# Healthcare-Robotics/assistive-gym

Hardware: NVIDIA H100
Metric: env-steps/sec FeedingJaco-v1 @batch4096 (higher is better)
Workload: dtype f32

## Files before the change

assistive_gym_b200/csrc/ag_bathing.cuh:

```cuda
#pragma once
#include "ag_task.cuh"
#include "../../include/agphys.h"

struct BathDev {
  AgBathingParams P;
  int *male, *iteration, *task_success, *total_targets;
  float* action;
  float* targets;
  int* alive;
  int* target_link;
  float* target_local;
  float* dist_part;
  int n_slots;
};

AG_HDN inline void bathing_pre_body(int e, const SimDev& S, const KP& p) {
  const BathDev& B = *(const BathDev*)p.p1;
  const float* act = (const float*)p.p0 + (size_t)e * (7 + p.i0);
  B.iteration[e] += 1;
  arm_action_targets(S, e, act, B.action, B.P.arm_links, B.P.arm_lower, B.P.arm_upper, B.P.action_multiplier, B.P.frame_skip);
}

AG_HDN inline void bathing_dist_body(int tid, const SimDev& S, const KP& p) {
  const int N = S.N;
  const BathDev& B = *(const BathDev*)p.p1;
  int e = tid % N, slot = tid / N;
  bool male = B.male[e] != 0;
  int c0 = male ? B.P.human_col0_m : B.P.human_col0_f, nc = male ? B.P.human_ncol_m : B.P.human_ncol_f;
  float best = 5.0f;
  if (slot < nc) {
    int ch = c0 + slot;
    int lt = AG_LDG(S.body_link0 + B.P.tool_body), nlt = AG_LDG(S.body_nlinks + B.P.tool_body);
    for (int l = lt; l < lt + nlt; l++) {
      int t0 = AG_LDG(S.link_col0 + l), tn = AG_LDG(S.link_ncol + l);
      for (int ct = t0; ct < t0 + tn; ct++) {
        NpOut out[4];
        int ca = ct < ch ? ct : ch, cb = ct < ch ? ch : ct;
        if (narrow_pair(S, e, ca, cb, 5.0f, false, out)) best = fminf(best, out[0].d);
      }
    }
  }
  B.dist_part[(size_t)slot * N + e] = best;
}

AG_HDN inline void bathing_track_body(int tid, const SimDev& S, const KP& p) {
  const int N = S.N;
  const BathDev& B = *(const BathDev*)p.p1;
  const int e = tid % N, t = tid / N;
  const int link = B.target_link[(size_t)t * N + e];
  if (link < 0) return;
  st3(B.targets, t, N, e, ld3(S.lpos, link, N, e) + qrot(ld4(S.lquat, link, N, e), ld3(B.target_local, t, N, e)));
}

// ... 49 lines not shown
```

assistive_gym_b200/csrc/ag_device.cuh:

```cuda
#pragma once
#include <string.h>
#include "ag_math.cuh"
#include "ag_types.h"

AG_HD float ld1(const float* p, int item, int N, int e) { return p[(size_t)item * N + e]; }
AG_HD void st1(float* p, int item, int N, int e, float v) { p[(size_t)item * N + e] = v; }
AG_HD f3 ld3(const float* p, int item, int N, int e) {
  size_t b = (size_t)item * 3 * N + e;
  return f3(p[b], p[b + N], p[b + 2 * (size_t)N]);
}
AG_HD void st3(float* p, int item, int N, int e, f3 v) {
  size_t b = (size_t)item * 3 * N + e;
  p[b] = v.x; p[b + N] = v.y; p[b + 2 * (size_t)N] = v.z;
}
AG_HD q4 ld4(const float* p, int item, int N, int e) {
  size_t b = (size_t)item * 4 * N + e;
  return q4(p[b], p[b + N], p[b + 2 * (size_t)N], p[b + 3 * (size_t)N]);
}
AG_HD void st4(float* p, int item, int N, int e, q4 v) {
  size_t b = (size_t)item * 4 * N + e;
  p[b] = v.x; p[b + N] = v.y; p[b + 2 * (size_t)N] = v.z; p[b + 3 * (size_t)N] = v.w;
}
AG_HD f3 tv3(const float* p, int i) { return f3(AG_LDG(p + 3 * i), AG_LDG(p + 3 * i + 1), AG_LDG(p + 3 * i + 2)); }
AG_HD q4 tv4(const float* p, int i) { return q4(AG_LDG(p + 4 * i), AG_LDG(p + 4 * i + 1), AG_LDG(p + 4 * i + 2), AG_LDG(p + 4 * i + 3)); }
// ... 50 lines not shown
  f3 hw(fabsf(R.m[0]) * h.x + fabsf(R.m[1]) * h.y + fabsf(R.m[2]) * h.z + r,
        fabsf(R.m[3]) * h.x + fabsf(R.m[4]) * h.y + fabsf(R.m[5]) * h.z + r,
        fabsf(R.m[6]) * h.x + fabsf(R.m[7]) * h.y + fabsf(R.m[8]) * h.z + r);
  st3(S.cmin, c, N, e, ctr - hw); st3(S.cmax, c, N, e, ctr + hw);
}
AG_HDN inline void linkaabb_body(int tid, const SimDev& S, const KP& p) {
  const int N = S.N;
  int e = tid % N, i = tid / N;
  int k = AG_LDG((const int*)p.p0 + i);
  int c0 = AG_LDG(S.link_col0 + k), ncl = AG_LDG(S.link_ncol + k);
  f3 mn(1e30f, 1e30f, 1e30f), mx(-1e30f, -1e30f, -1e30f);
  for (int c = c0; c < c0 + ncl; c++) { mn = fmin3(mn, ld3(S.cmin, c, N, e)); mx = fmax3(mx, ld3(S.cmax, c, N, e)); }
  st3(S.lmin, k, N, e, mn); st3(S.lmax, k, N, e, mx);
}

AG_HD bool aabb_ov(f3 amin, f3 amax, f3 bmin, f3 bmax, float m) {
  return !(amin.x > bmax.x + m || bmin.x > amax.x + m || amin.y > bmax.y + m || bmin.y > amax.y + m ||
           amin.z > bmax.z + m || bmin.z > amax.z + m);
}

AG_HD void seg_origin(d3 a, d3 b, double& u, double& v) {
  d3 ab = b - a;
  double t = -dot(a, ab), den = dot(ab, ab);
  if (t <= 0.0 || den <= 0.0) { u = 1.0; v = 0.0; return; }
  if (t >= den) { u = 0.0; v = 1.0; return; }
  v = t / den; u = 1.0 - v;
}
AG_HD void tri_origin(d3 a, d3 b, d3 c, double& u, double& v, double& w) {
  d3 ab = b - a, ac = c - a;
  double d1 = -dot(ab, a), d2 = -dot(ac, a);
// ... 26 lines not shown
  int bi = 0; float best = -3.0e38f;
  const int ng = (n + 3) >> 2;
  const float* p = vq + (size_t)g0 * 12;
  for (int g = 0; g < ng; g++, p += 12) {
    vq4 X = ldq4(p), Y = ldq4(p + 4), Z = ldq4(p + 8);
    float d0 = d.x * X.x + d.y * Y.x + d.z * Z.x, d1 = d.x * X.y + d.y * Y.y + d.z * Z.y;
    float d2 = d.x * X.z + d.y * Y.z + d.z * Z.z, d3v = d.x * X.w + d.y * Y.w + d.z * Z.w;
    if (d0 > best) { best = d0; bi = 4 * g; }
    if (d1 > best) { best = d1; bi = 4 * g + 1; }
    if (d2 > best) { best = d2; bi = 4 * g + 2; }
    if (d3v > best) { best = d3v; bi = 4 * g + 3; }
  }
  return bi < n ? bi : 0;
}

AG_HDN inline bool gjk_cores(const float* verts, const float* vq, int va0, int ga0, int nA, int vb0, int gb0, int nB, const m3& R, f3 t,
                             f3& pa, f3& pb, f3& nrm, float& dist) {
  d3 W[4]; f3 PA[4], PB[4];
  int IA[4], IB[4];
  double lam[4] = {1.0, 0.0, 0.0, 0.0};
  int n = 0;
  d3 v = to_d3(mul(R, tv3(verts, va0)) + t) - to_d3(tv3(verts, vb0));
  if (dot(v, v) < 1e-20) v = d3(1.0, 0.0, 0.0);
  bool overlap = false;
  double lower_bound = 0.0;
  for (int it = 0; it < 32; it++) {
    f3 vf = to_f3(v);
    f3 da = mulT(R, -vf);
    int ia = support4(vq, ga0, nA, da), ib = support4(vq, gb0, nB, vf);
    f3 sa = mul(R, tv3(verts, va0 + ia)) + t;
    f3 sb = tv3(verts, vb0 + ib);
    d3 w = to_d3(sa) - to_d3(sb);
    double vv = dot(v, v);
    double vw = dot(v, w);
    if (n > 0 && vw > 0.0) lower_bound = fmax(lower_bound, vw / sqrt(vv));
    if (n > 0 && vv - vw <= 1e-10 * vv) break;
    bool dup = false;
    for (int i = 0; i < n; i++) if (IA[i] == ia && IB[i] == ib) dup = true;
    if (dup) break;
    W[n] = w; PA[n] = sa; PB[n] = sb; IA[n] = ia; IB[n] = ib; n++;
    if (n == 1) { lam[0] = 1.0; }
    else if (n == 2) {
      double u, s; seg_origin(W[0], W[1], u, s);
      if (s <= 0.0) { n = 1; lam[0] = 1.0; }
      else if (u <= 0.0) { W[0] = W[1]; PA[0] = PA[1]; PB[0] = PB[1]; IA[0] = IA[1]; IB[0] = IB[1]; n = 1; lam[0] = 1.0; }
      else { lam[0] = u; lam[1] = s; }
    } else if (n == 3) {
      double l3[3]; tri_origin(W[0], W[1], W[2], l3[0], l3[1], l3[2]);
      int m = 0;
      for (int i = 0; i < 3; i++) if (l3[i] > 0.0) { W[m] = W[i]; PA[m] = PA[i]; PB[m] = PB[i]; IA[m] = IA[i]; IB[m] = IB[i]; lam[m] = l3[i]; m++; }
      n = m;
    } else {
      double bestd = 1e300; int bf = -1; double bl[3] = {0.0, 0.0, 0.0};
      double bestd_all = 1e300; int bf_all = 0; double bla[3] = {1.0, 0.0, 0.0};
      bool any_out = false;
      for (int f = 0; f < 4; f++) {
        int i0 = (f == 3) ? 1 : 0, i1 = (f == 0) ? 1 : ((f == 1) ? 2 : 3), i2 = (f == 0) ? 2 : ((f == 1) ? 3 : ((f == 2) ? 1 : 2)), i3 = (f == 0) ? 3 : ((f == 1) ? 1 : ((f == 2) ? 2 : 0));
        d3 a = W[i0], b = W[i1], c = W[i2], d = W[i3];
        d3 nn = cross(b - a, c - a);
        double sp = -dot(a, nn), sd = dot(d - a, nn);
        double nl = sqrt(dot(nn, nn));
        double tol_d = 1e-9 * nl * sqrt(dot(d - a, d - a)), tol_p = 1e-9 * nl * sqrt(dot(a, a));
        bool inside = (sp * sd > 0.0) && (fabs(sd) > tol_d) && (fabs(sp) > tol_p);
        double u, s, r; tri_origin(a, b, c, u, s, r);
        d3 pt = a * u + b * s + c * r;
        double dd = dot(pt, pt);
        if (dd < bestd_all) { bestd_all = dd; bf_all = f; bla[0] = u; bla[1] = s; bla[2] = r; }
        if (inside) continue;
        any_out = true;
        if (dd < bestd) { bestd = dd; bf = f; bl[0] = u; bl[1] = s; bl[2] = r; }
      }
      if (!any_out) {
        if (lower_bound <= 1e-7) { overlap = true; break; }
        bf = bf_all; bl[0] = bla[0]; bl[1] = bla[1]; bl[2] = bla[2];
      }
      int f = bf;
      int id[3];
      id[0] = (f == 3) ? 1 : 0; id[1] = (f == 0) ? 1 : ((f == 1) ? 2 : 3); id[2] = (f == 0) ? 2 : ((f == 1) ? 3 : ((f == 2) ? 1 : 2));
      d3 tw[3]; f3 ta[3], tb[3]; int tia[3], tib[3];
      for (int i = 0; i < 3; i++) { tw[i] = W[id[i]]; ta[i] = PA[id[i]]; tb[i] = PB[id[i]]; tia[i] = IA[id[i]]; tib[i] = IB[id[i]]; }
      int m = 0;
      for (int i = 0; i < 3; i++) if (bl[i] > 0.0) { W[m] = tw[i]; PA[m] = ta[i]; PB[m] = tb[i]; IA[m] = tia[i]; IB[m] = tib[i]; lam[m] = bl[i]; m++; }
      n = m;
    }
    d3 nv(0.0, 0.0, 0.0);
    for (int i = 0; i < n; i++) nv = nv + W[i] * lam[i];
    v = nv;
    if (dot(v, v) <= 1e-16) { overlap = true; break; }
  }
  if (overlap) return true;
  d3 qa(0.0, 0.0, 0.0), qb(0.0, 0.0, 0.0);
  for (int i = 0; i < n; i++) { qa = qa + to_d3(PA[i]) * lam[i]; qb = qb + to_d3(PB[i]) * lam[i]; }
  d3 d = qa - qb;
  double dn = sqrt(dot(d, d));
  pa = to_f3(qa); pb = to_f3(qb);
  dist = (float)dn;
  nrm = dn > 0.0 ? to_f3(d * (1.0 / dn)) : f3(0.f, 0.f, 1.f);
  return false;
}

AG_HDN inline void pen_faces(const SimDev& S, int va0, int nA, int pa0, int npA, int vb0, int nB, int pb0, int npB,
                             const m3& R, f3 t, f3& pa, f3& pb, f3& nrm, float& dist) {
  float best = -1e30f; bool found = false;
  for (int k = 0; k < npA; k++) {
    f3 nl; float dl; ld_plane(S.planes, pa0 + k, nl, dl);
    f3 n = mul(R, nl); float d = dl + dot(n, t);
    int jb = 0; float mn = dot(n, tv3(S.verts, vb0));
// ... 1 lines not shown
    float sep = mn - d;
    if (sep > best) { best = sep; found = true; nrm = -n; pb = tv3(S.verts, vb0 + jb); pa = pb - n * sep; }
  }
  for (int k = 0; k < npB; k++) {
    f3 n; float d; ld_plane(S.planes, pb0 + k, n, d);
    f3 nl = mulT(R, n);
    int ja = 0; float mn = dot(nl, tv3(S.verts, va0));
    for (int j = 1; j < nA; j++) { float x = dot(nl, tv3(S.verts, va0 + j)); if (x < mn) { mn = x; ja = j; } }
    float sep = mn + dot(n, t) - d;
    if (sep > best) { best = sep; found = true; nrm = n; pa = mul(R, tv3(S.verts, va0 + ja)) + t; pb = pa - n * sep; }
  }
  if (!found) { nrm = f3(0.f, 0.f, 1.f); pa = mul(R, tv3(S.verts, va0)) + t; pb = tv3(S.verts, vb0); best = 0.f; }
  dist = fminf(best, 0.f);
}

struct CandSet { NpOut c[4]; int n; };
struct CandSel {
  NpOut prim; NpOut pool[12]; int np;
};

AG_HDN inline void face_cands(const SimDev& S, int vv0, int nV, float rV, bool v_is_a, int p0, int np, float rP,
                              const m3& R, f3 t, f3 n_to_v, float d_primary, float tol, float max_dist, CandSel& cs) {
  int kf = -1; float best = 0.98f; f3 nf; float df = 0.f;
  for (int k = 0; k < np; k++) {
    f3 n; float d; ld_plane(S.planes, p0 + k, n, d);
    if (!v_is_a) { f3 nw = mul(R, n); d = d + dot(nw, t); n = nw; }
    float al = dot(n, n_to_v);
    if (al > best) { best = al; kf = k; nf = n; df = d; }
  }
  if (kf < 0) return;
  for (int i = 0; i < nV; i++) {
    f3 v = tv3(S.verts, vv0 + i);
    if (v_is_a) v = mul(R, v) + t;
    float h = dot(nf, v) - df;
    float d = h - rV - rP;
    if (d > d_primary + tol || d > max_dist) continue;
    f3 proj = v - nf * h;
    bool inside = true;
    for (int k = 0; k < np; k++) {
      if (k == kf) continue;
      f3 n; float dd; ld_plane(S.planes, p0 + k, n, dd);
      if (!v_is_a) { f3 nw = mul(R, n); dd = dd + dot(nw, t); n = nw; }
      if (dot(n, proj) - dd > 1e-6f) { inside = false; break; }
    }
    if (!inside) continue;
    if (cs.np >= 12) {
      int wi = 0; for (int q = 1; q < 12; q++) if (cs.pool[q].d > cs.pool[wi].d) wi = q;
      if (d >= cs.pool[wi].d) continue;
      cs.np = 12;
      NpOut& o = cs.pool[wi];
      f3 on_v = v - nf * rV, on_f = proj + nf * rP;
      if (v_is_a) { o.pa = on_v; o.pb = on_f; o.n = nf; } else { o.pa = on_f; o.pb = on_v; o.n = -nf; }
      o.d = d;
      continue;
    }
    NpOut& o = cs.pool[cs.np++];
    f3 on_v = v - nf * rV, on_f = proj + nf * rP;
    if (v_is_a) { o.pa = on_v; o.pb = on_f; o.n = nf; } else { o.pa = on_f; o.pb = on_v; o.n = -nf; }
    o.d = d;
  }
}

AG_HDN inline int select_cands(const CandSel& cs, NpOut* out) {
  if (cs.np == 0) { out[0] = cs.prim; return 1; }
  bool used[12];
  int first = 0;
  for (int i = 0; i < 12; i++) used[i] = i >= cs.np;
  for (int i = 1; i < cs.np; i++) if (cs.pool[i].d < cs.pool[first].d) first = i;
  int nc = 0; out[nc++] = cs.pool[first]; used[first] = true;
  while (nc < 4) {
    int bi = -1; float bd = 1e-8f;
    for (int i = 0; i < cs.np; i++) {
      if (used[i]) continue;
      float md = 1e30f;
      for (int k = 0; k < nc; k++) { f3 d = cs.pool[i].pa - out[k].pa; md = fminf(md, dot(d, d)); }
      if (md > bd) { bd = md; bi = i; }
    }
    if (bi < 0) break;
    used[bi] = true; out[nc++] = cs.pool[bi];
  }
  return nc;
}

AG_HDN inline int narrow_pair(const SimDev& S, int e, int ca, int cb, float max_dist, bool manifold, NpOut* out) {
  const int N = S.N;
  int ta = AG_LDG(S.col_type + ca), tb = AG_LDG(S.col_type + cb);
  float ra = AG_LDG(S.col_radius + ca), rb = AG_LDG(S.col_radius + cb);
  int ka = AG_LDG(S.col_link + ca), kb = AG_LDG(S.col_link + cb);
  int va0 = AG_LDG(S.col_v0 + ca), nA = AG_LDG(S.col_nv + ca), vb0 = AG_LDG(S.col_v0 + cb), nB = AG_LDG(S.col_nv + cb);
  int pa0 = AG_LDG(S.col_p0 + ca), npA = AG_LDG(S.col_np + ca), pb0 = AG_LDG(S.col_p0 + cb), npB = AG_LDG(S.col_np + cb);
  f3 posA = ld3(S.lpos, ka, N, e), posB = ld3(S.lpos, kb, N, e);
  q4 qA = ld4(S.lquat, ka, N, e), qB = ld4(S.lquat, kb, N, e);
  CandSel cs; cs.np = 0;
  int nout;
  if (ta == 3 || tb == 3) {
    if (ta == tb) return 0;
    bool flip = (ta == 3);
    q4 qP = flip ? qA : qB, qV = flip ? qB : qA;
    f3 pP = flip ? posA : posB, pV = flip ? posB : posA;
    m3 R = mul(transpose(qmat(qP)), qmat(qV));
    f3 t = qrot_inv(qP, pV - pP);
    int vv0 = flip ? vb0 : va0, nV = flip ? nB : nA; float rv = flip ? rb : ra;
    f3 pn; float pd; ld_plane(S.planes, flip ? pa0 : pb0, pn, pd);
    int j = 0; float mn = 1e30f;
    for (int i = 0; i < nV; i++) { float x = dot(pn, mul(R, tv3(S.verts, vv0 + i)) + t); if (x < mn) { mn = x; j = i; } }
    float d = mn - pd - rv;
    if (d > max_dist) return 0;
    f3 vj = mul(R, tv3(S.verts, vv0 + j)) + t;
    cs.prim.pa = vj - pn * rv; cs.prim.pb = vj - pn * (mn - pd); cs.prim.n = pn; cs.prim.d = d;
    if (manifold && nV > 1) face_cands(S, vv0, nV, rv, true, flip ? pa0 : pb0, 1, 0.f, R, t, pn, d, max_dist * 0.5f, max_dist, cs);
    nout = select_cands(cs, out);
    m3 RP = qmat(qP);
    for (int i = 0; i < nout; i++) {
      f3 a = mul(RP, out[i].pa) + pP, b = mul(RP, out[i].pb) + pP, n = mul(RP, out[i].n);
      if (!flip) { out[i].pa = a; out[i].pb = b; out[i].n = n; }
      else { out[i].pa = b; out[i].pb = a; out[i].n = -n; }
    }
    return nout;
  }
  m3 RB = qmat(qB);
  m3 R = mul(transpose(RB), qmat(qA));
  f3 t = mulT(RB, posA - posB);
  f3 pa, pb, nrm; float dist = 0.f;
  bool ov = gjk_cores(S.verts, S.vertq, va0, AG_LDG(S.col_g0 + ca), nA, vb0, AG_LDG(S.col_g0 + cb), nB, R, t, pa, pb, nrm, dist);
  if (ov) pen_faces(S, va0, nA, pa0, npA, vb0, nB, pb0, npB, R, t, pa, pb, nrm, dist);
  float d = dist - ra - rb;
  if (d > max_dist) return 0;
  cs.prim.n = nrm; cs.prim.pa = pa - nrm * ra; cs.prim.pb = pb + nrm * rb; cs.prim.d = d;
  if (manifold) {
    if (npB > 0 && nA > 1) face_cands(S, va0, nA, ra, true, pb0, npB, rb, R, t, nrm, d, max_dist * 0.5f, max_dist, cs);
    if (npA > 0 && nB > 1) face_cands(S, vb0, nB, rb, false, pa0, npA, ra, R, t, -nrm, d, max_dist * 0.5f, max_dist, cs);
  }
  nout = select_cands(cs, out);
  for (int i = 0; i < nout; i++) {
    out[i].pa = mul(RB, out[i].pa) + posB; out[i].pb = mul(RB, out[i].pb) + posB; out[i].n = mul(RB, out[i].n);
  }
  return nout;
}

AG_HD int ag_atomic_inc(int* p) {
#if defined(__CUDA_ARCH__)
  return atomicAdd(p, 1);
#else
  int v = *p; *p = v + 1; return v;
#endif
}
AG_HD int ag_atomic_add(int* p, int k) {
#if defined(__CUDA_ARCH__)
  return atomicAdd(p, k);
#else
  int v = *p; *p = v + k; return v;
#endif
// ... 25 lines not shown
    }
  }
}

AG_HDN inline void csort_body(int tid, const SimDev& S, const KP&) {
  const int N = S.N;
  int e = tid % N, cs = tid / N;
  int n = S.cand_count[e]; if (n > S.maxcand) n = S.maxcand;
  if (cs >= n) return;
  unsigned w = S.cand[(size_t)cs * N + e];
  int rank = 0;
  for (int j = 0; j < n; j++) rank += (S.cand[(size_t)j * N + e] < w) ? 1 : 0;
  S.cand_s[(size_t)rank * N + e] = w;
}

AG_HDN inline void narrow_body(int tid, const SimDev& S, const KP&) {
  const int N = S.N;
  int e = tid % N, cs = tid / N;
  int ncand = S.cand_count[e]; if (ncand > S.maxcand) ncand = S.maxcand;
  if (cs >= ncand) return;
  unsigned pk = S.cand_s[(size_t)cs * N + e] & 0xffffffu;
  int ca = (int)(pk / (unsigned)S.nc), cb = (int)(pk % (unsigned)S.nc);
  float thr = S.contact_thr * fminf(AG_LDG(S.col_thresh + ca), AG_LDG(S.col_thresh + cb));
  NpOut out[4];
  int n = narrow_pair(S, e, ca, cb, thr, true, out);
  for (int i = 0; i < n; i++) {
    int slot = ag_atomic_inc(S.c_count + e);
    if (slot >= S.maxraw) continue;
    S.c_key[(size_t)slot * N + e] = pk * 4u + (unsigned)i;
    float* c = S.c_data + (size_t)slot * AG_CFR * N + e;
    c[(size_t)CF_PAX * N] = out[i].pa.x; c[(size_t)CF_PAY * N] = out[i].pa.y; c[(size_t)CF_PAZ * N] = out[i].pa.z;
    c[(size_t)CF_PBX * N] = out[i].pb.x; c[(size_t)CF_PBY * N] = out[i].pb.y; c[(size_t)CF_PBZ * N] = out[i].pb.z;
    c[(size_t)CF_NX * N] = out[i].n.x; c[(size_t)CF_NY * N] = out[i].n.y; c[(size_t)CF_NZ * N] = out[i].n.z;
    c[(size_t)CF_DIST * N] = out[i].d;
  }
}

AG_HD void contact_refs(const SimDev& S, int e, unsigned key, int& refA, int& refB);
AG_HDN inline void sort_body(int tid, const SimDev& S, const KP&) {
  const int N = S.N;
  int e = tid % N, slot = tid / N;
  int cnt = S.c_count[e];
  int n = cnt < S.maxraw ? cnt : S.maxraw;
  if (slot == 0 && ((cnt > S.maxc) || (S.cand_count[e] > S.maxcand))) S.overflow[e] = 1;
  if (slot >= n) return;
  unsigned key = S.c_key[(size_t)slot * N + e];
  int rank = 0;
  for (int j = 0; j < n; j++) rank += (S.c_key[(size_t)j * N + e] < key) ? 1 : 0;
  if (rank >= S.maxc) return;
  S.s_key[(size_t)rank * N + e] = key;
// ... 248 lines not shown
```

assistive_gym_b200/csrc/ag_readback.cuh:

```cuda
#pragma once
#include <string.h>
#include "ag_task.cuh"

AG_HDN inline void gather_body(int tid, const SimDev& S, const KP& p) {
  const int N = S.N;
  int e = tid % N, j = tid / N;
  int comp = p.i0, K = p.i0 * p.i1;
  int item = ((const int*)p.p2)[j / comp], c = j % comp;
  ((float*)p.p1)[(size_t)e * K + j] = ((const float*)p.p0)[((size_t)item * comp + c) * N + e];
}
AG_HDN inline void scatter_body(int tid, const SimDev& S, const KP& p) {
  const int N = S.N;
  int e = tid % N, j = tid / N;
  if (p.p3 && !((const int*)p.p3)[e]) return;
  int comp = p.i0, K = p.i0 * p.i1;
  int item = ((const int*)p.p2)[j / comp], c = j % comp;
  ((float*)p.p1)[((size_t)item * comp + c) * N + e] = ((const float*)p.p0)[(size_t)e * K + j];
}

AG_HDN inline void linkstate_body(int tid, const SimDev& S, const KP& p) {
  const int N = S.N;
  int e = tid % N, j = tid / N, n = p.i1;
  int k = ((const int*)p.p2)[j];
  float* o = (float*)p.p1 + ((size_t)e * n + j) * 20;
// ... 47 lines not shown
  int ba = p.i0, bb = p.i1, max_pts = p.i2; float dist = p.f0;
  int a0 = AG_LDG(S.body_link0 + ba), an = AG_LDG(S.body_nlinks + ba), b0 = AG_LDG(S.body_link0 + bb), bn = AG_LDG(S.body_nlinks + bb);
  int n = 0;
  if (S.body_mode[(size_t)ba * N + e] == 0 || S.body_mode[(size_t)bb * N + e] == 0) { ((int*)p.p2)[e] = 0; return; }
  for (int la = a0; la < a0 + an; la++) {
    int nca = AG_LDG(S.link_ncol + la); if (!nca) continue;
    f3 lamin = ld3(S.lmin, la, N, e), lamax = ld3(S.lmax, la, N, e);
    for (int lb = b0; lb < b0 + bn; lb++) {
      int ncb = AG_LDG(S.link_ncol + lb); if (!ncb) continue;
      if (!aabb_ov(lamin, lamax, ld3(S.lmin, lb, N, e), ld3(S.lmax, lb, N, e), dist)) continue;
      int ca0 = AG_LDG(S.link_col0 + la), cb0 = AG_LDG(S.link_col0 + lb);
      for (int ca = ca0; ca < ca0 + nca; ca++) {
        f3 amin = ld3(S.cmin, ca, N, e), amax = ld3(S.cmax, ca, N, e);
        for (int cb = cb0; cb < cb0 + ncb; cb++) {
          if (!aabb_ov(amin, amax, ld3(S.cmin, cb, N, e), ld3(S.cmax, cb, N, e), dist)) continue;
          NpOut out[4];
          if (!narrow_pair(S, e, ca, cb, dist, false, out)) continue;
          if (n < max_pts) write_contact((float*)p.p1 + ((size_t)e * max_pts + n) * 13, la, lb, out[0].pa, out[0].pb, out[0].n, out[0].d, 0.f);
          n++;
        }
      }
    }
  }
  ((int*)p.p2)[e] = n;
}
```

assistive_gym_b200/csrc/ag_task.cuh:

```cuda
#pragma once
#include "ag_device.cuh"

AG_HD unsigned long long xorshift64s(unsigned long long& s) {
  s ^= s >> 12; s ^= s << 25; s ^= s >> 27;
  return s * 2685821657736338717ull;
}
AG_HD float rng_uniform(unsigned long long& s) { return (float)(xorshift64s(s) >> 40) * (1.0f / 16777216.0f); }

AG_HD void link_com_pose(const SimDev& S, int e, int k, f3& pos, q4& quat) {
  const int N = S.N;
  q4 q = ld4(S.lquat, k, N, e);
  pos = ld3(S.lpos, k, N, e) + qrot(q, tv3(S.link_com, k));
  quat = qmul(q, tv4(S.link_iquat, k));
}
AG_HD f3 link_com(const SimDev& S, int e, int k) {
  const int N = S.N;
  return ld3(S.lpos, k, N, e) + qrot(ld4(S.lquat, k, N, e), tv3(S.link_com, k));
}

struct Frame { f3 p; q4 qi; };
AG_HD Frame body_frame(const SimDev& S, int e, int body) {
  Frame fr; q4 q;
  link_com_pose(S, e, AG_LDG(S.body_link0 + body), fr.p, q);
  fr.qi = qconj(q);
// ... 101 lines not shown
  const int N = S.N;
  float an = 0.f;
  for (int j = 0; j < 7; j++) { float a = action[(size_t)j * N + e]; an += a * a; }
  for (int j = 0; j < i0; j++) { float a = act[(size_t)e * (7 + i0) + 7 + j]; an += a * a; }
  return sqrtf(an);
}
AG_HD float episode_done(int iteration) { return iteration >= 200 ? 1.f : 0.f; }

AG_HD bool tool_within(const SimDev& S, int e, int col, int tool_link, float dist) {
  const int N = S.N;
  f3 pmin = ld3(S.cmin, col, N, e), pmax = ld3(S.cmax, col, N, e);
  if (!aabb_ov(pmin, pmax, ld3(S.lmin, tool_link, N, e), ld3(S.lmax, tool_link, N, e), dist)) return false;
  int c0 = AG_LDG(S.link_col0 + tool_link), ncl = AG_LDG(S.link_ncol + tool_link);
  for (int c = c0; c < c0 + ncl; c++) {
    if (!aabb_ov(pmin, pmax, ld3(S.cmin, c, N, e), ld3(S.cmax, c, N, e), dist)) continue;
    NpOut out[4];
    if (narrow_pair(S, e, col, c, dist, false, out)) return true;
  }
  return false;
}
AG_HD void send_far(const SimDev& S, int e, int body, unsigned long long& rs) {
  const int N = S.N;
  int l0 = AG_LDG(S.body_link0 + body);
  f3 far(1000.f + 1000.f * rng_uniform(rs), 1000.f + 1000.f * rng_uniform(rs), 1000.f + 1000.f * rng_uniform(rs));
  st3(S.base_pos, body, N, e, far); st4(S.base_quat, body, N, e, q4());
  st3(S.lpos, l0, N, e, far); st4(S.lquat, l0, N, e, q4());
}
```

assistive_gym_b200/csrc/agphys.cu:

```cuda
#include <stdio.h>
#include <stdlib.h>
#include <string.h>
#include <string>
#include <vector>
#include <algorithm>
#include "../../include/agphys.h"
#include "ag_device.cuh"
#include "ag_solver.cuh"
#include "ag_readback.cuh"
#include "ag_feeding.cuh"
#include "ag_bathing.cuh"
#include "ag_ik.cuh"
#include "ag_cloth.cuh"
#include "ag_dressing.cuh"
#include "ag_render.cuh"
#include "ag_scratch.cuh"
#include "ag_coop.cuh"
#include "ag_drinking.cuh"

#ifndef AG_CPU_EMU
#include <cuda_runtime.h>
#define AG_GLOBAL __global__
#else
#define AG_GLOBAL
// ... 2 lines not shown

static thread_local std::string g_err;
static int fail(const std::string& m) { g_err = m; return -1; }

#ifndef AG_CPU_EMU
#define AG_KERNEL(name, body)                                                   \
  __global__ void __launch_bounds__(128) name(SimDev S, KP p) {                 \
    int tid = blockIdx.x * blockDim.x + threadIdx.x;                            \
    if (tid < p.n) body(tid, S, p);                                             \
  }
#else
#define AG_KERNEL(name, body) \
  static void name(SimDev S, KP p) { for (int tid = 0; tid < p.n; tid++) body(tid, S, p); }
#endif

#ifndef AG_CPU_EMU
#define AG_KERNEL_B(name, body, minblocks)                                      \
  __global__ void __launch_bounds__(128, minblocks) name(SimDev S, KP p) {      \
    int tid = blockIdx.x * blockDim.x + threadIdx.x;                            \
    if (tid < p.n) body(tid, S, p);                                             \
  }
#else
#define AG_KERNEL_B(name, body, minblocks) AG_KERNEL(name, body)
#endif
AG_KERNEL(k_fk, fk_body)
AG_KERNEL(k_aabb, aabb_body)
AG_KERNEL(k_linkaabb, linkaabb_body)
AG_KERNEL(k_pairs, pairs_body)
AG_KERNEL(k_csort, csort_body)
AG_KERNEL_B(k_narrow, narrow_body, 3)
AG_KERNEL(k_sort, sort_body)
#define DYN_T 32
#ifndef AG_CPU_EMU
__global__ void __launch_bounds__(2 * DYN_T) k_dyn(SimDev S, KP p) {
  extern __shared__ float dyn_smem[];
  if (threadIdx.x < DYN_T) {
    const int t = blockIdx.x * DYN_T + threadIdx.x;
    if (t < p.i0) dyn_art_body(t, S, dyn_smem + threadIdx.x * p.i2, p.i3);
  } else {
    for (int t = blockIdx.x * DYN_T + threadIdx.x - DYN_T; t < p.i1; t += gridDim.x * DYN_T) dyn_free_body(t, S);
  }
}
#else
static void k_dyn(SimDev S, KP p) {
  std::vector<float> w((size_t)p.i2);
// ... 754 lines not shown
  LAUNCH(s, k_fk, (size_t)S.nb * N, z);
  if (s->cloth) {
    KP cs = kp0(); cs.p0 = s->C_dev; cs.i0 = s->cloth_sub;
    LAUNCH(s, k_cloth_snap, (size_t)s->C.ncl * N, cs);
  }
  KP a = kp0(); a.p0 = S.movcol; a.i0 = S.nmovcol;
  LAUNCH(s, k_aabb, (size_t)S.nmovcol * N, a);
  KP l = kp0(); l.p0 = S.movlink; l.i0 = S.nmovlink;
  LAUNCH(s, k_linkaabb, (size_t)S.nmovlink * N, l);
  dev_zero(s, S.c_count, sizeof(int) * N);
  dev_zero(s, S.cand_count, sizeof(int) * N);
  int Npad = (N + 31) / 32 * 32;
  KP c = kp0(); c.i0 = Npad;
  LAUNCH(s, k_pairs, (size_t)S.nslice * Npad, c);
  LAUNCH(s, k_csort, (size_t)S.maxcand * N, z);
  LAUNCH(s, k_narrow, (size_t)S.maxcand * N, z);
  LAUNCH(s, k_sort, (size_t)S.maxraw * N, z);
  {
    KP d = z; d.i0 = S.nart * N; d.i1 = S.nf * N; d.i3 = s->dyn_cap; d.i2 = dyn_scratch_words(d.i3);
#ifndef AG_CPU_EMU
    int nblk = std::max((d.i0 + DYN_T - 1) / DYN_T, (d.i1 + 8 * DYN_T - 1) / (8 * DYN_T));
    if (nblk > 0) {
      int ps = s->profiling ? prof_slot(s, "k_dyn") : -1;
      if (ps >= 0) prof_mark(s, ps, true);
      k_dyn<<<nblk, 2 * DYN_T, (size_t)(d.i0 > 0 ? DYN_T * d.i2 : 0) * sizeof(float), s->stream>>>(S, d);
      if (ps >= 0) prof_mark(s, ps, false);
      s->launches++;
    }
#else
    LAUNCH(s, k_dyn, (size_t)(S.nf + S.nart) * N, d);
#endif
// ... 1070 lines not shown
```

Baseline: 394,000.

## Cut narrow-phase register pressure with shared-memory candidate pool and streaming emit

Restructures the narrow-phase collision routine so the 12-entry face-candidate pool lives in per-thread shared memory rather than in registers or local memory. Output contacts are streamed through an emit functor instead of being staged in an NpOut[4] array. GJK simplex indexing is rewritten with unrolled select loops so the arrays can stay in registers. The narrow kernel moves to 64-thread blocks with a higher min-blocks launch bound, and closest-point-only callers use a pool-free path. This trades shared-memory capacity and more complex code for less local-memory spilling and higher occupancy.

```diff
diff --git a/assistive_gym_b200/csrc/ag_bathing.cuh b/assistive_gym_b200/csrc/ag_bathing.cuh
--- a/assistive_gym_b200/csrc/ag_bathing.cuh
+++ b/assistive_gym_b200/csrc/ag_bathing.cuh
@@ -34,9 +34,9 @@
     for (int l = lt; l < lt + nlt; l++) {
       int t0 = AG_LDG(S.link_col0 + l), tn = AG_LDG(S.link_ncol + l);
       for (int ct = t0; ct < t0 + tn; ct++) {
-        NpOut out[4];
+        NpOut c;
         int ca = ct < ch ? ct : ch, cb = ct < ch ? ch : ct;
-        if (narrow_pair(S, e, ca, cb, 5.0f, false, out)) best = fminf(best, out[0].d);
+        if (narrow_closest(S, e, ca, cb, 5.0f, c)) best = fminf(best, c.d);
       }
     }
   }
diff --git a/assistive_gym_b200/csrc/ag_device.cuh b/assistive_gym_b200/csrc/ag_device.cuh
--- a/assistive_gym_b200/csrc/ag_device.cuh
+++ b/assistive_gym_b200/csrc/ag_device.cuh
@@ -88,6 +88,9 @@
   st3(S.lmin, k, N, e, mn); st3(S.lmax, k, N, e, mx);
 }
 
+#ifndef AG_NARROW_STAT
+#define AG_NARROW_STAT(event, value) ((void)0)
+#endif
 AG_HD bool aabb_ov(f3 amin, f3 amax, f3 bmin, f3 bmax, float m) {
   return !(amin.x > bmax.x + m || bmin.x > amax.x + m || amin.y > bmax.y + m || bmin.y > amax.y + m ||
            amin.z > bmax.z + m || bmin.z > amax.z + m);
@@ -144,17 +147,44 @@
   return bi < n ? bi : 0;
 }
 
+struct Simplex {
+  f3 PA[4], PB[4];
+  int IA[4], IB[4];
+  double lam[4];
+  AG_HD d3 w(int i) const { return to_d3(PA[i]) - to_d3(PB[i]); }
+  AG_HD d3 w_at(int i) const {
+    f3 a = PA[0], b = PB[0];
+#pragma unroll
+    for (int j = 1; j < 4; j++) if (j == i) { a = PA[j]; b = PB[j]; }
+    return to_d3(a) - to_d3(b);
+  }
+  AG_HD void put(int m, f3 a, f3 b, int ia, int ib) {
+#pragma unroll
+    for (int j = 0; j < 4; j++) if (j == m) { PA[j] = a; PB[j] = b; IA[j] = ia; IB[j] = ib; }
+  }
+  AG_HD void take(int m, const Simplex& s, int i, double l) {
+#pragma unroll
+    for (int j = 0; j < 4; j++) if (j == m) { PA[j] = s.PA[i]; PB[j] = s.PB[i]; IA[j] = s.IA[i]; IB[j] = s.IB[i]; lam[j] = l; }
+  }
+};
+AG_HD int tet_face(int f, int k) {
+  if (k == 0) return (f == 3) ? 1 : 0;
+  if (k == 1) return (f == 0) ? 1 : ((f == 1) ? 2 : 3);
+  if (k == 2) return (f == 0) ? 2 : ((f == 1) ? 3 : ((f == 2) ? 1 : 2));
+  return (f == 0) ? 3 : ((f == 1) ? 1 : ((f == 2) ? 2 : 0));
+}
+
 AG_HDN inline bool gjk_cores(const float* verts, const float* vq, int va0, int ga0, int nA, int vb0, int gb0, int nB, const m3& R, f3 t,
                              f3& pa, f3& pb, f3& nrm, float& dist) {
-  d3 W[4]; f3 PA[4], PB[4];
-  int IA[4], IB[4];
-  double lam[4] = {1.0, 0.0, 0.0, 0.0};
+  Simplex sx;
+  sx.lam[0] = 1.0; sx.lam[1] = 0.0; sx.lam[2] = 0.0; sx.lam[3] = 0.0;
   int n = 0;
   d3 v = to_d3(mul(R, tv3(verts, va0)) + t) - to_d3(tv3(verts, vb0));
   if (dot(v, v) < 1e-20) v = d3(1.0, 0.0, 0.0);
   bool overlap = false;
   double lower_bound = 0.0;
   for (int it = 0; it < 32; it++) {
+    AG_NARROW_STAT(gjk_iter, it);
     f3 vf = to_f3(v);
     f3 da = mulT(R, -vf);
     int ia = support4(vq, ga0, nA, da), ib = support4(vq, gb0, nB, vf);
@@ -166,27 +196,28 @@
     if (n > 0 && vw > 0.0) lower_bound = fmax(lower_bound, vw / sqrt(vv));
     if (n > 0 && vv - vw <= 1e-10 * vv) break;
     bool dup = false;
-    for (int i = 0; i < n; i++) if (IA[i] == ia && IB[i] == ib) dup = true;
+#pragma unroll
+    for (int i = 0; i < 4; i++) if (i < n && sx.IA[i] == ia && sx.IB[i] == ib) dup = true;
     if (dup) break;
-    W[n] = w; PA[n] = sa; PB[n] = sb; IA[n] = ia; IB[n] = ib; n++;
-    if (n == 1) { lam[0] = 1.0; }
+    sx.put(n, sa, sb, ia, ib); n++;
+    if (n == 1) { sx.lam[0] = 1.0; }
     else if (n == 2) {
-      double u, s; seg_origin(W[0], W[1], u, s);
-      if (s <= 0.0) { n = 1; lam[0] = 1.0; }
-      else if (u <= 0.0) { W[0] = W[1]; PA[0] = PA[1]; PB[0] = PB[1]; IA[0] = IA[1]; IB[0] = IB[1]; n = 1; lam[0] = 1.0; }
-      else { lam[0] = u; lam[1] = s; }
+      double u, s; seg_origin(sx.w(0), sx.w(1), u, s);
+      if (s <= 0.0) { n = 1; sx.lam[0] = 1.0; }
+      else if (u <= 0.0) { sx.take(0, sx, 1, 1.0); n = 1; }
+      else { sx.lam[0] = u; sx.lam[1] = s; }
     } else if (n == 3) {
-      double l3[3]; tri_origin(W[0], W[1], W[2], l3[0], l3[1], l3[2]);
+      double l3[3]; tri_origin(sx.w(0), sx.w(1), sx.w(2), l3[0], l3[1], l3[2]);
       int m = 0;
-      for (int i = 0; i < 3; i++) if (l3[i] > 0.0) { W[m] = W[i]; PA[m] = PA[i]; PB[m] = PB[i]; IA[m] = IA[i]; IB[m] = IB[i]; lam[m] = l3[i]; m++; }
+#pragma unroll
+      for (int i = 0; i < 3; i++) if (l3[i] > 0.0) { sx.take(m, sx, i, l3[i]); m++; }
       n = m;
     } else {
       double bestd = 1e300; int bf = -1; double bl[3] = {0.0, 0.0, 0.0};
-      double bestd_all = 1e300; int bf_all = 0; double bla[3] = {1.0, 0.0, 0.0};
+      double bestd_all = 1e300; int bf_all = -1;
       bool any_out = false;
       for (int f = 0; f < 4; f++) {
-        int i0 = (f == 3) ? 1 : 0, i1 = (f == 0) ? 1 : ((f == 1) ? 2 : 3), i2 = (f == 0) ? 2 : ((f == 1) ? 3 : ((f == 2) ? 1 : 2)), i3 = (f == 0) ? 3 : ((f == 1) ? 1 : ((f == 2) ? 2 : 0));
-        d3 a = W[i0], b = W[i1], c = W[i2], d = W[i3];
+        d3 a = sx.w_at(tet_face(f, 0)), b = sx.w_at(tet_face(f, 1)), c = sx.w_at(tet_face(f, 2)), d = sx.w_at(tet_face(f, 3));
         d3 nn = cross(b - a, c - a);
         double sp = -dot(a, nn), sd = dot(d - a, nn);
         double nl = sqrt(dot(nn, nn));
@@ -195,32 +226,38 @@
         double u, s, r; tri_origin(a, b, c, u, s, r);
         d3 pt = a * u + b * s + c * r;
         double dd = dot(pt, pt);
-        if (dd < bestd_all) { bestd_all = dd; bf_all = f; bla[0] = u; bla[1] = s; bla[2] = r; }
+        if (dd < bestd_all) { bestd_all = dd; bf_all = f; }
         if (inside) continue;
         any_out = true;
         if (dd < bestd) { bestd = dd; bf = f; bl[0] = u; bl[1] = s; bl[2] = r; }
       }
       if (!any_out) {
         if (lower_bound <= 1e-7) { overlap = true; break; }
-        bf = bf_all; bl[0] = bla[0]; bl[1] = bla[1]; bl[2] = bla[2];
+        bf = bf_all < 0 ? 0 : bf_all; bl[0] = 1.0; bl[1] = 0.0; bl[2] = 0.0;
+        if (bf_all >= 0) tri_origin(sx.w_at(tet_face(bf, 0)), sx.w_at(tet_face(bf, 1)), sx.w_at(tet_face(bf, 2)), bl[0], bl[1], bl[2]);
       }
-      int f = bf;
-      int id[3];
-      id[0] = (f == 3) ? 1 : 0; id[1] = (f == 0) ? 1 : ((f == 1) ? 2 : 3); id[2] = (f == 0) ? 2 : ((f == 1) ? 3 : ((f == 2) ? 1 : 2));
-      d3 tw[3]; f3 ta[3], tb[3]; int tia[3], tib[3];
-      for (int i = 0; i < 3; i++) { tw[i] = W[id[i]]; ta[i] = PA[id[i]]; tb[i] = PB[id[i]]; tia[i] = IA[id[i]]; tib[i] = IB[id[i]]; }
+      Simplex fc;
+#pragma unroll
+      for (int k = 0; k < 3; k++) {
+        const int src = tet_face(bf, k);
+#pragma unroll
+        for (int j = 0; j < 4; j++) if (j == src) fc.take(k, sx, j, 0.0);
+      }
       int m = 0;
-      for (int i = 0; i < 3; i++) if (bl[i] > 0.0) { W[m] = tw[i]; PA[m] = ta[i]; PB[m] = tb[i]; IA[m] = tia[i]; IB[m] = tib[i]; lam[m] = bl[i]; m++; }
+#pragma unroll
+      for (int i = 0; i < 3; i++) if (bl[i] > 0.0) { sx.take(m, fc, i, bl[i]); m++; }
       n = m;
     }
     d3 nv(0.0, 0.0, 0.0);
-    for (int i = 0; i < n; i++) nv = nv + W[i] * lam[i];
+#pragma unroll
+    for (int i = 0; i < 4; i++) if (i < n) nv = nv + sx.w(i) * sx.lam[i];
     v = nv;
     if (dot(v, v) <= 1e-16) { overlap = true; break; }
   }
   if (overlap) return true;
   d3 qa(0.0, 0.0, 0.0), qb(0.0, 0.0, 0.0);
-  for (int i = 0; i < n; i++) { qa = qa + to_d3(PA[i]) * lam[i]; qb = qb + to_d3(PB[i]) * lam[i]; }
+#pragma unroll
+  for (int i = 0; i < 4; i++) if (i < n) { qa = qa + to_d3(sx.PA[i]) * sx.lam[i]; qb = qb + to_d3(sx.PB[i]) * sx.lam[i]; }
   d3 d = qa - qb;
   double dn = sqrt(dot(d, d));
   pa = to_f3(qa); pb = to_f3(qb);
@@ -252,23 +289,29 @@
   dist = fminf(best, 0.f);
 }
 
-struct CandSet { NpOut c[4]; int n; };
-struct CandSel {
-  NpOut prim; NpOut pool[12]; int np;
-};
-
-AG_HDN inline void face_cands(const SimDev& S, int vv0, int nV, float rV, bool v_is_a, int p0, int np, float rP,
-                              const m3& R, f3 t, f3 n_to_v, float d_primary, float tol, float max_dist, CandSel& cs) {
-  int kf = -1; float best = 0.98f; f3 nf; float df = 0.f;
+#define NARROW_POOL 12
+#define NARROW_POOL_WORDS (9 * NARROW_POOL + 1)
+struct FaceRef { f3 nf; float df, rV, rP; int v0; bool v_is_a; };
+AG_HD FaceRef face_ref(int v0, bool v_is_a, float rV, float rP) {
+  FaceRef F; F.nf = f3(0.f, 0.f, 0.f); F.df = 0.f; F.rV = rV; F.rP = rP; F.v0 = v0; F.v_is_a = v_is_a; return F;
+}
+
+AG_HDN inline void face_cands(const SimDev& S, int call, FaceRef& F, int nV, int p0, int np, const m3& R, f3 t, f3 n_to_v,
+                              float d_primary, float tol, float max_dist, float* pool, int& np_pool) {
+  int* pkey = (int*)pool;
+  float* pd = pool + NARROW_POOL;
+  const bool v_is_a = F.v_is_a;
+  int kf = -1; float best = 0.98f;
   for (int k = 0; k < np; k++) {
     f3 n; float d; ld_plane(S.planes, p0 + k, n, d);
     if (!v_is_a) { f3 nw = mul(R, n); d = d + dot(nw, t); n = nw; }
     float al = dot(n, n_to_v);
-    if (al > best) { best = al; kf = k; nf = n; df = d; }
+    if (al > best) { best = al; kf = k; F.nf = n; F.df = d; }
   }
   if (kf < 0) return;
+  const f3 nf = F.nf; const float df = F.df, rV = F.rV, rP = F.rP;
   for (int i = 0; i < nV; i++) {
-    f3 v = tv3(S.verts, vv0 + i);
+    f3 v = tv3(S.verts, F.v0 + i);
     if (v_is_a) v = mul(R, v) + t;
     float h = dot(nf, v) - df;
     float d = h - rV - rP;
@@ -282,45 +325,47 @@
       if (dot(n, proj) - dd > 1e-6f) { inside = false; break; }
     }
     if (!inside) continue;
-    if (cs.np >= 12) {
-      int wi = 0; for (int q = 1; q < 12; q++) if (cs.pool[q].d > cs.pool[wi].d) wi = q;
-      if (d >= cs.pool[wi].d) continue;
-      cs.np = 12;
-      NpOut& o = cs.pool[wi];
-      f3 on_v = v - nf * rV, on_f = proj + nf * rP;
-      if (v_is_a) { o.pa = on_v; o.pb = on_f; o.n = nf; } else { o.pa = on_f; o.pb = on_v; o.n = -nf; }
-      o.d = d;
-      continue;
-    }
-    NpOut& o = cs.pool[cs.np++];
+    int q = np_pool;
+    if (np_pool >= NARROW_POOL) {
+      q = 0; for (int r = 1; r < NARROW_POOL; r++) if (pd[r] > pd[q]) q = r;
+      if (d >= pd[q]) continue;
+    } else {
+      np_pool++;
+    }
     f3 on_v = v - nf * rV, on_f = proj + nf * rP;
-    if (v_is_a) { o.pa = on_v; o.pb = on_f; o.n = nf; } else { o.pa = on_f; o.pb = on_v; o.n = -nf; }
-    o.d = d;
-  }
-}
-
-AG_HDN inline int select_cands(const CandSel& cs, NpOut* out) {
-  if (cs.np == 0) { out[0] = cs.prim; return 1; }
-  bool used[12];
-  int first = 0;
-  for (int i = 0; i < 12; i++) used[i] = i >= cs.np;
-  for (int i = 1; i < cs.np; i++) if (cs.pool[i].d < cs.pool[first].d) first = i;
-  int nc = 0; out[nc++] = cs.pool[first]; used[first] = true;
-  while (nc < 4) {
-    int bi = -1; float bd = 1e-8f;
-    for (int i = 0; i < cs.np; i++) {
-      if (used[i]) continue;
-      float md = 1e30f;
-      for (int k = 0; k < nc; k++) { f3 d = cs.pool[i].pa - out[k].pa; md = fminf(md, dot(d, d)); }
-      if (md > bd) { bd = md; bi = i; }
-    }
-    if (bi < 0) break;
-    used[bi] = true; out[nc++] = cs.pool[bi];
-  }
-  return nc;
-}
-
-AG_HDN inline int narrow_pair(const SimDev& S, int e, int ca, int cb, float max_dist, bool manifold, NpOut* out) {
+    f3 pa = v_is_a ? on_v : on_f, pb = v_is_a ? on_f : on_v;
+    pkey[q] = (i << 1) | call;
+    pd[q] = d;
+    float* ppa = pool + 3 * NARROW_POOL + 3 * q;
+    float* ppb = pool + 6 * NARROW_POOL + 3 * q;
+    ppa[0] = pa.x; ppa[1] = pa.y; ppa[2] = pa.z;
+    ppb[0] = pb.x; ppb[1] = pb.y; ppb[2] = pb.z;
+  }
+}
+
+AG_HD f3 pool_pa(const float* pool, int q) {
+  const float* p = pool + 3 * NARROW_POOL + 3 * q;
+  return f3(p[0], p[1], p[2]);
+}
+AG_HD NpOut pool_contact(const float* pool, int q, const FaceRef& F0, const FaceRef& F1) {
+  const bool c1 = (((const int*)pool)[q] & 1) != 0;
+  const float* pb = pool + 6 * NARROW_POOL + 3 * q;
+  NpOut o;
+  o.pa = pool_pa(pool, q); o.pb = f3(pb[0], pb[1], pb[2]);
+  o.n = c1 ? -F1.nf : F0.nf;
+  o.d = pool[NARROW_POOL + q];
+  return o;
+}
+
+AG_HD NpOut np_world(const NpOut& c, const m3& Rw, f3 pw, bool flip) {
+  f3 a = mul(Rw, c.pa) + pw, b = mul(Rw, c.pb) + pw, n = mul(Rw, c.n);
+  NpOut o; o.d = c.d;
+  if (!flip) { o.pa = a; o.pb = b; o.n = n; } else { o.pa = b; o.pb = a; o.n = -n; }
+  return o;
+}
+
+template <class Emit>
+AG_HDN inline int narrow_pair(const SimDev& S, int e, int ca, int cb, float max_dist, float* pool, Emit& emit) {
   const int N = S.N;
   int ta = AG_LDG(S.col_type + ca), tb = AG_LDG(S.col_type + cb);
   float ra = AG_LDG(S.col_radius + ca), rb = AG_LDG(S.col_radius + cb);
@@ -329,15 +374,18 @@
   int pa0 = AG_LDG(S.col_p0 + ca), npA = AG_LDG(S.col_np + ca), pb0 = AG_LDG(S.col_p0 + cb), npB = AG_LDG(S.col_np + cb);
   f3 posA = ld3(S.lpos, ka, N, e), posB = ld3(S.lpos, kb, N, e);
   q4 qA = ld4(S.lquat, ka, N, e), qB = ld4(S.lquat, kb, N, e);
-  CandSel cs; cs.np = 0;
-  int nout;
+  NpOut prim;
+  m3 R, Rw; f3 t, pw; bool flip = false;
+  FaceRef F0, F1;
+  int np_pool = 0;
   if (ta == 3 || tb == 3) {
     if (ta == tb) return 0;
-    bool flip = (ta == 3);
+    flip = (ta == 3);
     q4 qP = flip ? qA : qB, qV = flip ? qB : qA;
     f3 pP = flip ? posA : posB, pV = flip ? posB : posA;
-    m3 R = mul(transpose(qmat(qP)), qmat(qV));
-    f3 t = qrot_inv(qP, pV - pP);
+    Rw = qmat(qP); pw = pP;
+    R = mul(transpose(Rw), qmat(qV));
+    t = qrot_inv(qP, pV - pP);
     int vv0 = flip ? vb0 : va0, nV = flip ? nB : nA; float rv = flip ? rb : ra;
     f3 pn; float pd; ld_plane(S.planes, flip ? pa0 : pb0, pn, pd);
     int j = 0; float mn = 1e30f;
@@ -345,35 +393,56 @@
     float d = mn - pd - rv;
     if (d > max_dist) return 0;
     f3 vj = mul(R, tv3(S.verts, vv0 + j)) + t;
-    cs.prim.pa = vj - pn * rv; cs.prim.pb = vj - pn * (mn - pd); cs.prim.n = pn; cs.prim.d = d;
-    if (manifold && nV > 1) face_cands(S, vv0, nV, rv, true, flip ? pa0 : pb0, 1, 0.f, R, t, pn, d, max_dist * 0.5f, max_dist, cs);
-    nout = select_cands(cs, out);
-    m3 RP = qmat(qP);
-    for (int i = 0; i < nout; i++) {
-      f3 a = mul(RP, out[i].pa) + pP, b = mul(RP, out[i].pb) + pP, n = mul(RP, out[i].n);
-      if (!flip) { out[i].pa = a; out[i].pb = b; out[i].n = n; }
-      else { out[i].pa = b; out[i].pb = a; out[i].n = -n; }
-    }
-    return nout;
-  }
-  m3 RB = qmat(qB);
-  m3 R = mul(transpose(RB), qmat(qA));
-  f3 t = mulT(RB, posA - posB);
-  f3 pa, pb, nrm; float dist = 0.f;
-  bool ov = gjk_cores(S.verts, S.vertq, va0, AG_LDG(S.col_g0 + ca), nA, vb0, AG_LDG(S.col_g0 + cb), nB, R, t, pa, pb, nrm, dist);
-  if (ov) pen_faces(S, va0, nA, pa0, npA, vb0, nB, pb0, npB, R, t, pa, pb, nrm, dist);
-  float d = dist - ra - rb;
-  if (d > max_dist) return 0;
-  cs.prim.n = nrm; cs.prim.pa = pa - nrm * ra; cs.prim.pb = pb + nrm * rb; cs.prim.d = d;
-  if (manifold) {
-    if (npB > 0 && nA > 1) face_cands(S, va0, nA, ra, true, pb0, npB, rb, R, t, nrm, d, max_dist * 0.5f, max_dist, cs);
-    if (npA > 0 && nB > 1) face_cands(S, vb0, nB, rb, false, pa0, npA, ra, R, t, -nrm, d, max_dist * 0.5f, max_dist, cs);
-  }
-  nout = select_cands(cs, out);
-  for (int i = 0; i < nout; i++) {
-    out[i].pa = mul(RB, out[i].pa) + posB; out[i].pb = mul(RB, out[i].pb) + posB; out[i].n = mul(RB, out[i].n);
-  }
-  return nout;
+    prim.pa = vj - pn * rv; prim.pb = vj - pn * (mn - pd); prim.n = pn; prim.d = d;
+    F0 = face_ref(vv0, true, rv, 0.f); F1 = F0;
+    if (pool && nV > 1) face_cands(S, 0, F0, nV, flip ? pa0 : pb0, 1, R, t, pn, d, max_dist * 0.5f, max_dist, pool, np_pool);
+  } else {
+    Rw = qmat(qB); pw = posB;
+    R = mul(transpose(Rw), qmat(qA));
+    t = mulT(Rw, posA - posB);
+    f3 pa, pb, nrm; float dist = 0.f;
+    bool ov = gjk_cores(S.verts, S.vertq, va0, AG_LDG(S.col_g0 + ca), nA, vb0, AG_LDG(S.col_g0 + cb), nB, R, t, pa, pb, nrm, dist);
+    if (ov) { AG_NARROW_STAT(pen_faces, 1); pen_faces(S, va0, nA, pa0, npA, vb0, nB, pb0, npB, R, t, pa, pb, nrm, dist); }
+    float d = dist - ra - rb;
+    if (d > max_dist) return 0;
+    prim.n = nrm; prim.pa = pa - nrm * ra; prim.pb = pb + nrm * rb; prim.d = d;
+    F0 = face_ref(va0, true, ra, rb); F1 = face_ref(vb0, false, rb, ra);
+    if (pool) {
+      if (npB > 0 && nA > 1) face_cands(S, 0, F0, nA, pb0, npB, R, t, nrm, d, max_dist * 0.5f, max_dist, pool, np_pool);
+      if (npA > 0 && nB > 1) face_cands(S, 1, F1, nB, pa0, npA, R, t, -nrm, d, max_dist * 0.5f, max_dist, pool, np_pool);
+    }
+  }
+  AG_NARROW_STAT(pool, np_pool);
+  if (np_pool == 0) { emit(0, np_world(prim, Rw, pw, flip)); return 1; }
+  const float* pd = pool + NARROW_POOL;
+  float* pmd = pool + 2 * NARROW_POOL;
+  int first = 0;
+  for (int i = 1; i < np_pool; i++) if (pd[i] < pd[first]) first = i;
+  for (int i = 0; i < np_pool; i++) pmd[i] = 1e30f;
+  unsigned used = 1u << first;
+  int nc = 0, cur = first;
+  for (;;) {
+    NpOut c = pool_contact(pool, cur, F0, F1);
+    emit(nc++, np_world(c, Rw, pw, flip));
+    if (nc == 4) break;
+    int bi = -1; float bd = 1e-8f;
+    for (int i = 0; i < np_pool; i++) {
+      if ((used >> i) & 1u) continue;
+      f3 dv = pool_pa(pool, i) - c.pa;
+      float md = fminf(pmd[i], dot(dv, dv));
+      pmd[i] = md;
+      if (md > bd) { bd = md; bi = i; }
+    }
+    if (bi < 0) break;
+    used |= 1u << bi; cur = bi;
+  }
+  return nc;
+}
+
+struct FirstContact { NpOut* c; AG_HD void operator()(int, const NpOut& x) const { *c = x; } };
+AG_HD bool narrow_closest(const SimDev& S, int e, int ca, int cb, float max_dist, NpOut& out) {
+  FirstContact k; k.c = &out;
+  return narrow_pair(S, e, ca, cb, max_dist, nullptr, k) > 0;
 }
 
 AG_HD int ag_atomic_inc(int* p) {
@@ -429,7 +498,21 @@
   S.cand_s[(size_t)rank * N + e] = w;
 }
 
-AG_HDN inline void narrow_body(int tid, const SimDev& S, const KP&) {
+struct RawContacts {
+  const SimDev* S; int e; unsigned pk;
+  AG_HD void operator()(int i, const NpOut& o) const {
+    const int N = S->N;
+    int slot = ag_atomic_inc(S->c_count + e);
+    if (slot >= S->maxraw) return;
+    S->c_key[(size_t)slot * N + e] = pk * 4u + (unsigned)i;
+    float* c = S->c_data + (size_t)slot * AG_CFR * N + e;
+    c[(size_t)CF_PAX * N] = o.pa.x; c[(size_t)CF_PAY * N] = o.pa.y; c[(size_t)CF_PAZ * N] = o.pa.z;
+    c[(size_t)CF_PBX * N] = o.pb.x; c[(size_t)CF_PBY * N] = o.pb.y; c[(size_t)CF_PBZ * N] = o.pb.z;
+    c[(size_t)CF_NX * N] = o.n.x; c[(size_t)CF_NY * N] = o.n.y; c[(size_t)CF_NZ * N] = o.n.z;
+    c[(size_t)CF_DIST * N] = o.d;
+  }
+};
+AG_HDN inline void narrow_body(int tid, const SimDev& S, float* pool) {
   const int N = S.N;
   int e = tid % N, cs = tid / N;
   int ncand = S.cand_count[e]; if (ncand > S.maxcand) ncand = S.maxcand;
@@ -437,18 +520,10 @@
   unsigned pk = S.cand_s[(size_t)cs * N + e] & 0xffffffu;
   int ca = (int)(pk / (unsigned)S.nc), cb = (int)(pk % (unsigned)S.nc);
   float thr = S.contact_thr * fminf(AG_LDG(S.col_thresh + ca), AG_LDG(S.col_thresh + cb));
-  NpOut out[4];
-  int n = narrow_pair(S, e, ca, cb, thr, true, out);
-  for (int i = 0; i < n; i++) {
-    int slot = ag_atomic_inc(S.c_count + e);
-    if (slot >= S.maxraw) continue;
-    S.c_key[(size_t)slot * N + e] = pk * 4u + (unsigned)i;
-    float* c = S.c_data + (size_t)slot * AG_CFR * N + e;
-    c[(size_t)CF_PAX * N] = out[i].pa.x; c[(size_t)CF_PAY * N] = out[i].pa.y; c[(size_t)CF_PAZ * N] = out[i].pa.z;
-    c[(size_t)CF_PBX * N] = out[i].pb.x; c[(size_t)CF_PBY * N] = out[i].pb.y; c[(size_t)CF_PBZ * N] = out[i].pb.z;
-    c[(size_t)CF_NX * N] = out[i].n.x; c[(size_t)CF_NY * N] = out[i].n.y; c[(size_t)CF_NZ * N] = out[i].n.z;
-    c[(size_t)CF_DIST * N] = out[i].d;
-  }
+  RawContacts out; out.S = &S; out.e = e; out.pk = pk;
+  AG_NARROW_STAT(cand, tid);
+  const int n = narrow_pair(S, e, ca, cb, thr, pool, out);
+  AG_NARROW_STAT(done, n);
 }
 
 AG_HD void contact_refs(const SimDev& S, int e, unsigned key, int& refA, int& refB);
diff --git a/assistive_gym_b200/csrc/ag_readback.cuh b/assistive_gym_b200/csrc/ag_readback.cuh
--- a/assistive_gym_b200/csrc/ag_readback.cuh
+++ b/assistive_gym_b200/csrc/ag_readback.cuh
@@ -85,9 +85,9 @@
         f3 amin = ld3(S.cmin, ca, N, e), amax = ld3(S.cmax, ca, N, e);
         for (int cb = cb0; cb < cb0 + ncb; cb++) {
           if (!aabb_ov(amin, amax, ld3(S.cmin, cb, N, e), ld3(S.cmax, cb, N, e), dist)) continue;
-          NpOut out[4];
-          if (!narrow_pair(S, e, ca, cb, dist, false, out)) continue;
-          if (n < max_pts) write_contact((float*)p.p1 + ((size_t)e * max_pts + n) * 13, la, lb, out[0].pa, out[0].pb, out[0].n, out[0].d, 0.f);
+          NpOut c;
+          if (!narrow_closest(S, e, ca, cb, dist, c)) continue;
+          if (n < max_pts) write_contact((float*)p.p1 + ((size_t)e * max_pts + n) * 13, la, lb, c.pa, c.pb, c.n, c.d, 0.f);
           n++;
         }
       }
diff --git a/assistive_gym_b200/csrc/ag_task.cuh b/assistive_gym_b200/csrc/ag_task.cuh
--- a/assistive_gym_b200/csrc/ag_task.cuh
+++ b/assistive_gym_b200/csrc/ag_task.cuh
@@ -139,8 +139,8 @@
   int c0 = AG_LDG(S.link_col0 + tool_link), ncl = AG_LDG(S.link_ncol + tool_link);
   for (int c = c0; c < c0 + ncl; c++) {
     if (!aabb_ov(pmin, pmax, ld3(S.cmin, c, N, e), ld3(S.cmax, c, N, e), dist)) continue;
-    NpOut out[4];
-    if (narrow_pair(S, e, col, c, dist, false, out)) return true;
+    NpOut out;
+    if (narrow_closest(S, e, col, c, dist, out)) return true;
   }
   return false;
 }
diff --git a/assistive_gym_b200/csrc/agphys.cu b/assistive_gym_b200/csrc/agphys.cu
--- a/assistive_gym_b200/csrc/agphys.cu
+++ b/assistive_gym_b200/csrc/agphys.cu
@@ -40,21 +40,24 @@
   static void name(SimDev S, KP p) { for (int tid = 0; tid < p.n; tid++) body(tid, S, p); }
 #endif
 
-#ifndef AG_CPU_EMU
-#define AG_KERNEL_B(name, body, minblocks)                                      \
-  __global__ void __launch_bounds__(128, minblocks) name(SimDev S, KP p) {      \
-    int tid = blockIdx.x * blockDim.x + threadIdx.x;                            \
-    if (tid < p.n) body(tid, S, p);                                             \
-  }
-#else
-#define AG_KERNEL_B(name, body, minblocks) AG_KERNEL(name, body)
-#endif
 AG_KERNEL(k_fk, fk_body)
 AG_KERNEL(k_aabb, aabb_body)
 AG_KERNEL(k_linkaabb, linkaabb_body)
 AG_KERNEL(k_pairs, pairs_body)
 AG_KERNEL(k_csort, csort_body)
-AG_KERNEL_B(k_narrow, narrow_body, 3)
+#define NARROW_T 64
+#ifndef AG_CPU_EMU
+__global__ void __launch_bounds__(NARROW_T, 6) k_narrow(SimDev S, KP p) {
+  __shared__ float pool[NARROW_T * NARROW_POOL_WORDS];
+  int tid = blockIdx.x * blockDim.x + threadIdx.x;
+  if (tid < p.n) narrow_body(tid, S, pool + threadIdx.x * NARROW_POOL_WORDS);
+}
+#else
+static void k_narrow(SimDev S, KP p) {
+  float pool[NARROW_POOL_WORDS];
+  for (int tid = 0; tid < p.n; tid++) narrow_body(tid, S, pool);
+}
+#endif
 AG_KERNEL(k_sort, sort_body)
 #define DYN_T 32
 #ifndef AG_CPU_EMU
@@ -839,7 +842,18 @@
   KP c = kp0(); c.i0 = Npad;
   LAUNCH(s, k_pairs, (size_t)S.nslice * Npad, c);
   LAUNCH(s, k_csort, (size_t)S.maxcand * N, z);
+#ifndef AG_CPU_EMU
+  {
+    KP kp = z; kp.n = S.maxcand * N;
+    int ps = s->profiling ? prof_slot(s, "k_narrow") : -1;
+    if (ps >= 0) prof_mark(s, ps, true);
+    k_narrow<<<(kp.n + NARROW_T - 1) / NARROW_T, NARROW_T, 0, s->stream>>>(S, kp);
+    if (ps >= 0) prof_mark(s, ps, false);
+    s->launches++;
+  }
+#else
   LAUNCH(s, k_narrow, (size_t)S.maxcand * N, z);
+#endif
   LAUNCH(s, k_sort, (size_t)S.maxraw * N, z);
   {
     KP d = z; d.i0 = S.nart * N; d.i1 = S.nf * N; d.i3 = s->dyn_cap; d.i2 = dyn_scratch_words(d.i3);
```

Measured after the change: 406,800, median of 6. 3.2% higher.
